# vovw/algonauts-2025

Hardware: AMD Instinct MI355X
Metric: TRs/sec trimodal encode to 1000 parcels (higher is better)
Workload: dtype bf16; 1 GPU; trimodal encode, precomputed bf16 feats, per GPU B=64 sequences (4 subjects x R=16) x T=1024, L*D=4096 per modality, hidden 3072, 8 layers, V=1000 parcels, n_output_timesteps=1024; forward only; global_batch=64, seq_len=1024, parallelism=dp1

## Files before the change

### algonauts-2025_amd/csrc/gemm.hip

```cpp
#include "gemm_common.h"

namespace {

constexpr int BK = 64;
typedef __attribute__((ext_vector_type(4))) short s16x4_tn;
constexpr int TRIBE_ROLE_EXT = 100;

namespace big {
constexpr int BM = 256, BN = 256;
constexpr int A_BYTES = BM * BK * 2;
constexpr int BUF_BYTES = 2 * A_BYTES;
constexpr int SMEM_BYTES = 2 * BUF_BYTES;
}

#define TRIBE_WAIT_VMCNT_(n) asm volatile("s_waitcnt vmcnt(" #n ")" ::: "memory")
#define TRIBE_WAIT_VMCNT(n) TRIBE_WAIT_VMCNT_(n)
#ifndef TRIBE_GEMM_VM_STEADY
#define TRIBE_GEMM_VM_STEADY 8
#endif

#ifdef TRIBE_GEMM_STAMPS
#define TRIBE_STAMP(var)                                                                  \
  do {                                                                                    \
    __builtin_amdgcn_sched_barrier(0);                                                    \
    asm volatile("s_memtime %0\n\ts_waitcnt lgkmcnt(0)" : "=s"(var)::"memory");           \
    __builtin_amdgcn_sched_barrier(0);                                                    \
  } while (0)
#define TRIBE_STAMP_ACC(slot, t_from, t_to) stamp_acc[slot] += (t_to) - (t_from)
#else
#define TRIBE_STAMP(var) do { } while (0)
#define TRIBE_STAMP_ACC(slot, t_from, t_to) do { } while (0)
#endif

template <int N> __device__ __forceinline__ void wait_vmcnt() { asm volatile("s_waitcnt vmcnt(%0)" ::"n"(N) : "memory"); }

struct SkSched {
  int tiles_dp;
  int rem_units;
  int q;
  int workers;
  float* ws;
  unsigned short second_worker[256];
};
constexpr int SK_SLOT_FLOATS = 256 * 256;

template <int OUT_BF16, int ROLE, int TN = 0, int NB = 4>
__global__ __launch_bounds__(512, 2) void gemm_nt_256x256x64(const tribe_gemm_desc g, int tiles_m, int tiles_n, const SkSched sk) {
  static_assert(NB >= 2 && NB <= 4 && (!TN || NB == 4), "tile columns: 128, 192 or 256; transposed operands: 256 only");
  constexpr int BM = big::BM, BN = 64 * NB, A_BYTES = big::A_BYTES, BUF_BYTES = A_BYTES + BN * BK * 2;
  constexpr int WN = 16 * NB;
  constexpr int VM_STEADY = NB == 4 ? TRIBE_GEMM_VM_STEADY : 4 + NB;
  extern __shared__ __attribute__((aligned(16))) char smem[];
#ifdef TRIBE_GEMM_STAMPS
  unsigned long long ts_entry = 0, ts_loop = 0, ts_end = 0;
  TRIBE_STAMP(ts_entry);
#endif
  const int tid = threadIdx.x;
  const int lane = tid & 63;
  const int wave = __builtin_amdgcn_readfirstlane(tid >> 6);
  const int wr = wave >> 2, wc = wave & 3;

  int tile_lin = (int)blockIdx.x, k_first = 0, nk = (int)(g.K / BK);
  bool partial = false;
  int sk_slot = 0;
  if constexpr (TN) {
    if ((int)blockIdx.x >= sk.tiles_dp) {
      const int sidx = (int)blockIdx.x - sk.tiles_dp;
      const bool second = sidx >= sk.workers;
      const int w = second ? (int)sk.second_worker[sidx - sk.workers] : sidx;
      const int u0 = w * sk.q;
      if (u0 >= sk.rem_units) return;
      const int run = min(sk.q, sk.rem_units - u0);
      const int t_loc = u0 / nk, x = u0 - t_loc * nk, first_len = min(run, nk - x);
      if (second && first_len >= run) return;
      tile_lin = sk.tiles_dp + t_loc + (second ? 1 : 0);
      k_first = second ? 0 : x;
      const int len = second ? run - first_len : first_len;
      partial = len != nk;
      nk = len;
      sk_slot = 2 * w + (second ? 1 : 0);
    }
  }
  int tm, tn;
  tile_coords(tile_lin, tiles_m, tiles_n, tm, tn);
  const int64_t m0 = (int64_t)tm * BM, n0 = (int64_t)tn * BN;

  const int64_t z = blockIdx.y;
  const int64_t b1 = z / g.batch0, b0 = z - b1 * g.batch0;
  const int64_t b1g = g.gather1 ? g.gather1[b1] : b1;
  const unsigned short* A = (const unsigned short*)g.A + (g.gather_a ? b1g : b1) * g.sA1 + b0 * g.sA0;
  const unsigned short* B = (const unsigned short*)g.B + (g.gather_b ? b1g : b1) * g.sB1 + b0 * g.sB0;

  const int srow = lane >> 3;
  const int schunk = (lane & 7) ^ srow;
#ifdef TRIBE_ABL_SAME_TILE
#define m0 ((int64_t)0)
#define n0 ((int64_t)0)
#endif
  const unsigned short* a_src[2][2];
  const unsigned short* b_src[NB];
  int a_lds[2][2], b_lds[NB];
#pragma unroll
  for (int h = 0; h < 2; ++h)
#pragma unroll
    for (int j = 0; j < 2; ++j) {
      if (TN) {
        const int piece = 8 * j + wave, krow = 4 * piece + (lane >> 4);
        const int lc = (lane & 15) ^ ((krow & 7) << 1);
        int64_t gm = m0 + (lc >> 3) * 128 + h * 64 + (lc & 7) * 8; gm = gm + 8 <= g.M ? gm : g.M - 8;
        int64_t gn = n0 + (lc >> 2) * 64 + h * 32 + (lc & 3) * 8; gn = gn + 8 <= g.N ? gn : g.N - 8;
        a_src[h][j] = A + (int64_t)krow * g.lda + gm;
        b_src[(2 * h + j) % NB] = B + (int64_t)krow * g.ldb + gn;
        a_lds[h][j] = h * 16384 + piece * 1024;
        b_lds[(2 * h + j) % NB] = A_BYTES + h * 16384 + piece * 1024;
      } else {
        const int ra = j * 128 + h * 64 + wave * 8;
        int64_t gr = m0 + ra + srow; gr = gr < g.M ? gr : g.M - 1;
        a_src[h][j] = A + gr * g.lda + schunk * 8;
        a_lds[h][j] = ra * 128;
      }
    }
  if (!TN) {
#pragma unroll
    for (int q = 0; q < NB; ++q) {
      const int rb = q * 64 + wave * 8;
      int64_t gc = n0 + rb + srow; gc = gc < g.N ? gc : g.N - 1;
      b_src[q] = B + gc * g.ldb + schunk * 8;
      b_lds[q] = A_BYTES + rb * 128;
    }
  }

#ifdef TRIBE_ABL_SAME_TILE
#undef m0
#undef n0
#endif
  auto stage = [&](int which, int buf, int kt) {
#ifdef TRIBE_ABL_NO_STAGE
    return;
#endif
    char* base = smem + buf * BUF_BYTES;
    const int64_t koff_a = TN ? (int64_t)kt * BK * g.lda : (int64_t)kt * BK;
    const int64_t koff_b = TN ? (int64_t)kt * BK * g.ldb : (int64_t)kt * BK;
    if (which == 0 || which == 3) {
      const int h = which == 3;
      __builtin_amdgcn_global_load_lds((gptr_t)(a_src[h][0] + koff_a), (lptr_t)(base + a_lds[h][0]), 16, 0, 0);
      __builtin_amdgcn_global_load_lds((gptr_t)(a_src[h][1] + koff_a), (lptr_t)(base + a_lds[h][1]), 16, 0, 0);
    } else {
#pragma unroll
      for (int q = 0; q < NB; ++q)
        __builtin_amdgcn_global_load_lds((gptr_t)(b_src[q] + koff_b), (lptr_t)(base + b_lds[q]), 16, 0, 0);
    }
  };

  f32x4_t acc[8][NB];
#pragma unroll
  for (int i = 0; i < 8; ++i)
#pragma unroll
    for (int j = 0; j < NB; ++j) acc[i][j] = f32x4_t{0.f, 0.f, 0.f, 0.f};

  const int frow = lane & 15, fq = lane >> 4;
  const int coff0 = ((fq ^ (frow & 7)) << 4), coff1 = (((4 + fq) ^ (frow & 7)) << 4);
  const int a_rd = (wr * 128 + frow) * 128;
#ifdef TRIBE_GEMM_NO_TACC
  constexpr int TACC = 0;
#else
  constexpr int TACC = TN ? 0 : 1;
#endif
  const int prow = TACC ? ((frow & 3) | ((frow & 4) << 1) | ((frow & 8) >> 1)) : frow;
  const int bcoff0 = ((fq ^ (prow & 7)) << 4), bcoff1 = (((4 + fq) ^ (prow & 7)) << 4);
  const int b_rd = A_BYTES + (wc * WN + prow) * 128;

  bf16x8_t fa[4][2], fb[NB][2];
#ifdef TRIBE_ABL_NO_LDSREAD
#pragma unroll
  for (int i = 0; i < 4; ++i)
#pragma unroll
    for (int k = 0; k < 2; ++k) {
      fa[i][k] = bf16x8_t{(short)(0x3c00 + lane), (short)0x3f80, (short)(0xbf00 + i), (short)0x3e00, (short)0xbe80, (short)0x3f00, (short)(0x3d00 + k), (short)0xbd00};
      if (i < NB) fb[i][k] = fa[i][k];
    }
#endif

  const int tq = frow >> 2, tp = frow & 3;
  const int t_row = 4 * fq + tq, t_sw = (t_row & 7) << 1;
  int ta_off[4], tb_off[2];
#pragma unroll
  for (int i = 0; i < 4; ++i) ta_off[i] = t_row * 256 + (((wr * 8 + 2 * i + (tp >> 1)) ^ t_sw) << 4) + (tp & 1) * 8;
#pragma unroll
  for (int j = 0; j < 2; ++j) tb_off[j] = A_BYTES + t_row * 256 + (((wc * 4 + 2 * j + (tp >> 1)) ^ t_sw) << 4) + (tp & 1) * 8;
  auto tr_frag = [&](const char* p) -> bf16x8_t {
    const s16x4_tn lo = __builtin_amdgcn_ds_read_tr16_b64_v4i16((__attribute__((address_space(3))) s16x4_tn*)(p));
    const s16x4_tn hi = __builtin_amdgcn_ds_read_tr16_b64_v4i16((__attribute__((address_space(3))) s16x4_tn*)(p + 16 * 256));
    bf16x8_t f;
#pragma unroll
    for (int e = 0; e < 4; ++e) { f[e] = lo[e]; f[4 + e] = hi[e]; }
    return f;
  };

#ifdef TRIBE_ABL_NO_LDSREAD
#define TRIBE_LDS_A(base, MH) _Pragma("unroll") for (int i = 0; i < 4; ++i) { asm volatile("" : "+v"(fa[i][0]), "+v"(fa[i][1])); }
#define TRIBE_LDS_B(base) _Pragma("unroll") for (int j = 0; j < NB; ++j) { asm volatile("" : "+v"(fb[j][0]), "+v"(fb[j][1])); }
#else
#define TRIBE_LDS_A(base, MH)                                                                  \
  _Pragma("unroll") for (int i = 0; i < 4; ++i) {                                              \
    if (TN) {                                                                                  \
      fa[i][0] = tr_frag((base) + (MH) * 16384 + ta_off[i]);                                   \
      fa[i][1] = tr_frag((base) + (MH) * 16384 + ta_off[i] + 32 * 256);                        \
    } else {                                                                                   \
      fa[i][0] = *(const bf16x8_t*)((base) + a_rd + (MH) * 8192 + i * 2048 + coff0);           \
      fa[i][1] = *(const bf16x8_t*)((base) + a_rd + (MH) * 8192 + i * 2048 + coff1);           \
    }                                                                                          \
  }
// ... 23 lines not shown
  }
#endif
#ifdef TRIBE_GEMM_PRIO_FLIPS
#define TRIBE_PRIO_UP() __builtin_amdgcn_s_setprio(1)
#define TRIBE_PRIO_DOWN() __builtin_amdgcn_s_setprio(0)
#else
#define TRIBE_PRIO_UP() __builtin_amdgcn_sched_barrier(0)
#define TRIBE_PRIO_DOWN() __builtin_amdgcn_sched_barrier(0)
#endif
#define TRIBE_PHASE_SYNC_MMA(MH)                           \
  asm volatile("s_waitcnt lgkmcnt(0)" ::: "memory");       \
  __builtin_amdgcn_sched_barrier(0);                       \
  TRIBE_STAMP(ts2);                                        \
  __builtin_amdgcn_s_barrier();                            \
  TRIBE_STAMP(ts3);                                        \
  TRIBE_PRIO_UP();                                         \
  TRIBE_MMA(MH)                                            \
  TRIBE_PRIO_DOWN();                                       \
  TRIBE_STAMP(ts4);                                        \
  __builtin_amdgcn_s_barrier();                            \
  TRIBE_STAMP(ts5);                                        \
  TRIBE_STAMP_ACC(1, ts1, ts2); TRIBE_STAMP_ACC(2, ts2, ts3); TRIBE_STAMP_ACC(3, ts3, ts4); TRIBE_STAMP_ACC(4, ts4, ts5);

#ifdef TRIBE_GEMM_NO_KROT
  const int krot = 0;
#else
  const int krot = ((tn & 7) + (tm & 3)) % nk;
#endif
  auto ktile = [&](int t) { const int k = t + krot; return k_first + (k >= nk ? k - nk : k); };
#ifdef TRIBE_GEMM_STAMPS
  unsigned long long ts0 = 0, ts1 = 0, ts2 = 0, ts3 = 0, ts4 = 0, ts5 = 0;
  unsigned long long stamp_acc[5] = {0, 0, 0, 0, 0};
#endif

  stage(0, 0, ktile(0)); stage(1, 0, ktile(0)); stage(3, 0, ktile(0));
  if (nk > 1) {
    stage(0, 1, ktile(1)); stage(1, 1, ktile(1));
    wait_vmcnt<2 + NB>();
  } else {
    wait_vmcnt<0>();
  }
  __builtin_amdgcn_s_barrier();
  if (wr == 1) __builtin_amdgcn_s_barrier();
#if !defined(TRIBE_GEMM_PRIO_FLIPS) && !defined(TRIBE_ABL_NO_PRIO)
  if (wr == 1) __builtin_amdgcn_s_setprio(1);
#endif

  TRIBE_STAMP(ts_loop);
  for (int t = 0; t < nk; ++t) {
    const int cur = t & 1;
    const char* base = smem + cur * BUF_BYTES;
    TRIBE_STAMP(ts0);
    TRIBE_LDS_B(base)
    TRIBE_LDS_A(base, 0)
    TRIBE_STAMP(ts1);
    TRIBE_STAMP_ACC(0, ts0, ts1);
    if (t + 1 < nk) { stage(3, cur ^ 1, ktile(t + 1)); wait_vmcnt<VM_STEADY>(); } else { wait_vmcnt<0>(); }
    TRIBE_PHASE_SYNC_MMA(0)
    TRIBE_STAMP(ts0);
    TRIBE_LDS_A(base, 1)
    TRIBE_STAMP(ts1);
    TRIBE_STAMP_ACC(0, ts0, ts1);
    if (t + 2 < nk) {
      const int k2 = ktile(t + 2);
// ... 9 lines not shown
  TRIBE_STAMP(ts_end);
#ifdef TRIBE_GEMM_STAMPS
  if (g.gadd == nullptr && g.gadd_index != nullptr && lane == 0 && blockIdx.y == 0) {
    unsigned long long* dbg = (unsigned long long*)g.gadd_index + ((size_t)blockIdx.x * 8 + wave) * 8;
    for (int i = 0; i < 5; ++i) dbg[i] = stamp_acc[i];
  }
#endif
#undef TRIBE_LDS_A
#undef TRIBE_LDS_B
#undef TRIBE_MMA
#undef TRIBE_PHASE_SYNC_MMA

  const EpiCtx ctx = make_epi_ctx(g, b1, b0, b1g);
  if constexpr (TN && !OUT_BF16) {
    if (partial) {
      float* slot = sk.ws + (int64_t)sk_slot * SK_SLOT_FLOATS + tid * 4;
      static_for<8 * NB>([&](auto t) {
        constexpr int i = decltype(t)::value / NB, j = decltype(t)::value % NB;
        *(f32x4_t*)(slot + (i * NB + j) * 2048) = acc[i][j];
      });
      return;
    }
  }
  constexpr bool ROLE_EPI = TACC && (ROLE == TRIBE_ROLE_QKV || ROLE == TRIBE_ROLE_FF1 || ROLE == TRIBE_ROLE_OUT_PROJ || ROLE == TRIBE_ROLE_FF2);
  if constexpr (ROLE_EPI) {
    epilogue_role<OUT_BF16, ROLE, 8, NB, TACC>(g, acc, m0 + wr * 128, n0 + wc * WN, lane, smem + wave * (4 * NB * 1024));
  } else if (epilogue_fast_ok<(ROLE == TRIBE_ROLE_EXT)>(g, ctx) && n0 + BN <= g.N) {
    epilogue_fast<OUT_BF16, 8, NB, (ROLE == TRIBE_ROLE_EXT), TACC>(g, ctx, acc, m0 + wr * 128, n0 + wc * WN, lane, smem + wave * (4 * NB * 1024));
  } else {
    static_for<8 * NB>([&](auto t) {
      constexpr int i = decltype(t)::value / NB, j = decltype(t)::value % NB;
      epilogue_tile16<OUT_BF16, (ROLE == TRIBE_ROLE_EXT), TACC>(g, ctx, acc[i][j], m0 + wr * 128 + i * 16, n0 + wc * WN + j * 16, lane);
    });
  }
#ifdef TRIBE_GEMM_STAMPS
  TRIBE_STAMP(ts1);
  asm volatile("s_waitcnt vmcnt(0)" ::: "memory");
  TRIBE_STAMP(ts2);
  if (g.gadd == nullptr && g.gadd_index != nullptr && lane == 0 && blockIdx.y == 0) {
    unsigned long long* dbg = (unsigned long long*)g.gadd_index + ((size_t)blockIdx.x * 8 + wave) * 8;
    dbg[5] = ts_loop - ts_entry; dbg[6] = ts1 - ts_end; dbg[7] = ts2 - ts_end;
  }
#endif
}

__global__ __launch_bounds__(512) void streamk_reduce_kernel(const tribe_gemm_desc g, int tiles_m, int tiles_n, const SkSched sk) {
  const int tid = threadIdx.x, lane = tid & 63, wave = tid >> 6, wr = wave >> 2, wc = wave & 3;
// ... 614 lines not shown




#ifndef TRIBE_GEMM_PART
#define TRIBE_GEMM_PART -1
#endif
#define TRIBE_GEMM_HAS_PART(p) (TRIBE_GEMM_PART < 0 || TRIBE_GEMM_PART == (p))

namespace tribe_gemm_detail {
enum { KIND_SMALL = 0, KIND_BIG = 1, KIND_RING = 2, KIND_BIG4W = 3 };
#define TRIBE_GEMM_PAIRS(X)                                                                                            \
  X(0, 1, TRIBE_ROLE_GENERIC) X(1, 0, TRIBE_ROLE_GENERIC) X(2, 1, TRIBE_ROLE_EXT) X(3, 0, TRIBE_ROLE_EXT)              \
  X(4, 0, TRIBE_ROLE_PROJECTOR) X(5, 1, TRIBE_ROLE_QKV) X(6, 0, TRIBE_ROLE_ATTN_SCORES) X(7, 1, TRIBE_ROLE_ATTN_PV)    \
  X(8, 0, TRIBE_ROLE_OUT_PROJ) X(9, 1, TRIBE_ROLE_FF1) X(10, 0, TRIBE_ROLE_FF2) X(11, 0, TRIBE_ROLE_VOXEL_HEAD)
void launch_big4(int pair, dim3 grid, hipStream_t s, const tribe_gemm_desc* d, int tiles_m, int tiles_n);
void launch_big4_tn(int bf, dim3 grid, hipStream_t s, const tribe_gemm_desc* d, int tiles_m, int tiles_n, const SkSched& sk);
void launch_big3(int pair, dim3 grid, hipStream_t s, const tribe_gemm_desc* d, int tiles_m, int tiles_n);
void launch_ring(int pair, dim3 grid, hipStream_t s, const tribe_gemm_desc* d, int tiles_m, int tiles_n, int splits, float* ws);
void launch_splitk_epilogue(int bf, hipStream_t s, const tribe_gemm_desc* d, int splits, const float* ws);
void launch_4w(int pair, dim3 grid, hipStream_t s, const tribe_gemm_desc* d, int tiles_m, int tiles_n);
void launch_small(int pair, dim3 grid, hipStream_t s, const tribe_gemm_desc* d, int tiles_m, int tiles_n);

template <auto KERNEL, int THREADS, int SMEM, class... Extra>
static void launch_k(dim3 grid, hipStream_t s, const tribe_gemm_desc* d, int tiles_m, int tiles_n, const Extra&... extra) {
  static bool attr_done[64] = {};
  int dev = 0;
  (void)hipGetDevice(&dev);
  if (dev < 0 || dev >= 64 || !attr_done[dev]) {
    (void)hipFuncSetAttribute((const void*)KERNEL, hipFuncAttributeMaxDynamicSharedMemorySize, SMEM);
    if (dev >= 0 && dev < 64) attr_done[dev] = true;
  }
  hipLaunchKernelGGL(KERNEL, grid, dim3(THREADS, 1, 1), SMEM, s, *d, tiles_m, tiles_n, extra...);
}
inline const SkSched& no_stream_k() {
  static const SkSched none = [] { SkSched k{}; k.tiles_dp = 0x7fffffff; return k; }();
  return none;
}
#define TRIBE_GEMM_TABLE(NAME)                                                                                         \
  void NAME(int pair, dim3 grid, hipStream_t s, const tribe_gemm_desc* d, int tiles_m, int tiles_n) {                  \
    switch (pair) {                                                                                                    \
      TRIBE_GEMM_PAIRS(TRIBE_GEMM_CASE_##NAME)                                                                         \
      default: break;                                                                                                  \
    }                                                                                                                  \
  }
#if TRIBE_GEMM_HAS_PART(0)
#define TRIBE_GEMM_CASE_launch_big4(idx, bf, role) \
  case idx: launch_k<gemm_nt_256x256x64<bf, role, 0, 4>, 512, big::SMEM_BYTES>(grid, s, d, tiles_m, tiles_n, no_stream_k()); break;
TRIBE_GEMM_TABLE(launch_big4)
void launch_big4_tn(int bf, dim3 grid, hipStream_t s, const tribe_gemm_desc* d, int tiles_m, int tiles_n, const SkSched& sk) {
  if (bf) launch_k<gemm_nt_256x256x64<1, TRIBE_ROLE_GENERIC, 1, 4>, 512, big::SMEM_BYTES>(grid, s, d, tiles_m, tiles_n, sk);
  else launch_k<gemm_nt_256x256x64<0, TRIBE_ROLE_GENERIC, 1, 4>, 512, big::SMEM_BYTES>(grid, s, d, tiles_m, tiles_n, sk);
}
#endif
#if TRIBE_GEMM_HAS_PART(1)
#define TRIBE_GEMM_CASE_launch_big3(idx, bf, role) \
  case idx: launch_k<gemm_nt_256x256x64<bf, role, 0, 3>, 512, 2 * (big::A_BYTES + 192 * BK * 2)>(grid, s, d, tiles_m, tiles_n, no_stream_k()); break;
TRIBE_GEMM_TABLE(launch_big3)
#endif
#if TRIBE_GEMM_HAS_PART(2)
#define TRIBE_GEMM_CASE_launch_ring(idx, bf, role) \
  case idx: launch_k<gemm_nt_ring128<bf, role>, 512, ring::SMEM_BYTES>(grid, s, d, tiles_m, tiles_n, splits, ws); break;
void launch_ring(int pair, dim3 grid, hipStream_t s, const tribe_gemm_desc* d, int tiles_m, int tiles_n, int splits, float* ws) {
  switch (pair) {
    TRIBE_GEMM_PAIRS(TRIBE_GEMM_CASE_launch_ring)
    default: break;
  }
}
void launch_splitk_epilogue(int bf, hipStream_t s, const tribe_gemm_desc* d, int splits, const float* ws) {
  const int64_t threads = d->M * (d->N / 4);
  const dim3 grid((unsigned)((threads + 255) / 256));
  if (bf) hipLaunchKernelGGL(splitk_epilogue_kernel<1>, grid, dim3(256), 0, s, *d, splits, ws);
  else hipLaunchKernelGGL(splitk_epilogue_kernel<0>, grid, dim3(256), 0, s, *d, splits, ws);
}
#define TRIBE_GEMM_CASE_launch_small(idx, bf, role) \
  case idx: launch_k<gemm_nt_128x128x64<bf, role>, 256, small::SMEM_BYTES>(grid, s, d, tiles_m, tiles_n); break;
TRIBE_GEMM_TABLE(launch_small)
#endif
#if TRIBE_GEMM_HAS_PART(3)
#ifdef TRIBE_GEMM_STAMPS4W
// ... 268 lines not shown
    TRIBE_REQUIRE(nz == 1 && !d->rowadd && !d->gadd && !d->aux && (d->act == TRIBE_ACT_NONE || d->act == TRIBE_ACT_GELU),
                  "tribe_gemm_bf16: c_bf16 / row_sumsq / row_scale need an un-batched launch with plain operators");
    TRIBE_REQUIRE(d->ldc % 4 == 0 && ((uintptr_t)d->C % 16) == 0 && (!d->bias || ((uintptr_t)d->bias % 16) == 0) &&
                      (!d->res || (d->ldres % 4 == 0 && ((uintptr_t)d->res % 16) == 0)) && (!d->res_scale || ((uintptr_t)d->res_scale % 16) == 0),
                  "tribe_gemm_bf16: c_bf16 / row_sumsq / row_scale need 16-byte aligned operands");
    TRIBE_REQUIRE((!d->c_bf16 && !d->row_sumsq) || d->c_dtype == TRIBE_F32, "tribe_gemm_bf16: c_bf16 / row_sumsq accompany an f32 C");
    TRIBE_REQUIRE(!d->c_bf16 || (d->ld_c_bf16 >= d->N && d->ld_c_bf16 % 4 == 0 && ((uintptr_t)d->c_bf16 % 8) == 0), "tribe_gemm_bf16: bad c_bf16");
  }
  const tribe_gemm_detail::GemmPlan plan = tribe_gemm_detail::gemm_plan(d);
  if (d->c_bf16 || d->row_sumsq || d->row_scale) {
    TRIBE_REQUIRE(d->N % plan.bn == 0, "tribe_gemm_bf16: c_bf16 / row_sumsq / row_scale need N (%lld) to be a multiple of the tile width %d",
                  (long long)d->N, plan.bn);
    TRIBE_REQUIRE(!d->row_sumsq || d->ld_row_sumsq >= d->N / plan.sumsq_cols, "tribe_gemm_bf16: ld_row_sumsq must cover N / %d slots (tribe_gemm_sumsq_slots)",
                  plan.sumsq_cols);
  }
  if (d->trans_ab) {
    TRIBE_REQUIRE(d->M >= 8 && d->N >= 8 && d->M % 8 == 0 && d->N % 8 == 0 && d->lda >= d->M && d->ldb >= d->N,
                  "tribe_gemm_bf16: trans_ab takes At [K, M] and Bt [K, N] with M and N multiples of 8 and lda >= M, ldb >= N");
    TRIBE_REQUIRE(!d->aux && d->act != TRIBE_ACT_SWIGLU && d->act != TRIBE_ACT_GLU && d->act != TRIBE_ACT_SILU && d->act != TRIBE_ACT_GELU_BWD &&
                      d->act != TRIBE_ACT_EXP2 && d->act != TRIBE_ACT_MUL_AUX && !d->gather_a && !d->gather_b,
                  "tribe_gemm_bf16: trans_ab supports the plain epilogue operators and no operand gather");
  }
  const int64_t tiles_m = (d->M + plan.bm - 1) / plan.bm, tiles_n = (d->N + plan.bn - 1) / plan.bn;
  TRIBE_REQUIRE(tiles_m * tiles_n < (1ll << 31) && nz < 65536, "tribe_gemm_bf16: grid too large");

  dim3 grid((unsigned)(tiles_m * tiles_n), (unsigned)nz, 1);
  hipStream_t s = (hipStream_t)stream;
  const int role = (d->role >= 0 && d->role < TRIBE_ROLE_COUNT) ? d->role : TRIBE_ROLE_GENERIC;
  const double flops = 2.0 * (double)d->M * (double)d->N * (double)d->K * (double)nz;
  const int slot = prof_before(role, flops, s);
  const bool bf = d->c_dtype == TRIBE_BF16;
  if (d->trans_ab) {
    SkSched sk = tribe_gemm_detail::no_stream_k();
    if (d->stream_k) {
      TRIBE_REQUIRE(!bf && nz == 1 && d->bias_mode == TRIBE_BIAS_NONE && d->act == TRIBE_ACT_NONE && !d->res && !d->rowadd && !d->gadd,
                    "tribe_gemm_bf16: stream_k takes a plain un-batched f32 product");
      grid.x = tribe_gemm_detail::plan_stream_k((int)(tiles_m * tiles_n), (int)(d->K / BK), &sk);
      if (sk.tiles_dp < tiles_m * tiles_n) {
        const int64_t need = (int64_t)2 * sk.workers * SK_SLOT_FLOATS * 4;
        TRIBE_REQUIRE(d->stream_k_ws && d->stream_k_ws_bytes >= need && ((uintptr_t)d->stream_k_ws % 16) == 0,
                      "tribe_gemm_bf16: stream_k needs a 16-byte aligned workspace of %lld bytes (tribe_gemm_stream_k_workspace_bytes)", (long long)need);
        sk.ws = (float*)d->stream_k_ws;
      }
    }
    tribe_gemm_detail::launch_big4_tn(bf ? 1 : 0, grid, s, d, (int)tiles_m, (int)tiles_n, sk);
    if (sk.tiles_dp < tiles_m * tiles_n)
      hipLaunchKernelGGL(streamk_reduce_kernel, dim3((unsigned)(tiles_m * tiles_n - sk.tiles_dp)), dim3(512), 0, s, *d, (int)tiles_m, (int)tiles_n, sk);
// ... 19 lines not shown
    default: break;
    }
  }
  using namespace tribe_gemm_detail;
  if (plan.kind == KIND_BIG && (pair == 5 || pair == 8 || pair == 9 || pair == 10) && !takes_role_epilogue(d, plan)) pair = bf ? 0 : 1;
  if (plan.kind == KIND_BIG4W) launch_4w(pair, grid, s, d, (int)tiles_m, (int)tiles_n);
  else if (plan.kind == KIND_BIG && plan.bn == 192) launch_big3(pair, grid, s, d, (int)tiles_m, (int)tiles_n);
  else if (plan.kind == KIND_BIG) launch_big4(pair, grid, s, d, (int)tiles_m, (int)tiles_n);
  else if (plan.kind == KIND_RING && plan.splits > 1) {
    const int64_t need = (int64_t)plan.splits * d->M * d->N * 4;
    TRIBE_REQUIRE(d->stream_k_ws && d->stream_k_ws_bytes >= need && ((uintptr_t)d->stream_k_ws % 16) == 0,
                  "tribe_gemm_bf16: this launch is split over K: stream_k_ws must hold %lld bytes (tribe_gemm_stream_k_workspace_bytes)", (long long)need);
    TRIBE_REQUIRE(tiles_m * tiles_n * plan.splits < (1ll << 31) && d->M * (d->N / 4) < (1ll << 39), "tribe_gemm_bf16: grid too large");
    grid.x = (unsigned)(tiles_m * tiles_n * plan.splits);
    launch_ring(pair, grid, s, d, (int)tiles_m, (int)tiles_n, plan.splits, (float*)d->stream_k_ws);
    launch_splitk_epilogue(bf ? 1 : 0, s, d, plan.splits, (const float*)d->stream_k_ws);
  } else if (plan.kind == KIND_RING) launch_ring(pair, grid, s, d, (int)tiles_m, (int)tiles_n, 1, nullptr);
  else launch_small(pair, grid, s, d, (int)tiles_m, (int)tiles_n);
  prof_after(slot, s);
  TRIBE_LAUNCH_CHECK();
  return 0;
}

extern "C" int tribe_gemm_stream_k_plan(int32_t tiles, int32_t nk, int32_t* out) {
  TRIBE_REQUIRE(tiles > 0 && nk > 0 && out != nullptr, "tribe_gemm_stream_k_plan: bad argument");
  SkSched sk;
  const unsigned grid = tribe_gemm_detail::plan_stream_k(tiles, nk, &sk);
  out[0] = sk.tiles_dp; out[1] = sk.rem_units; out[2] = sk.q; out[3] = sk.workers;
  for (int i = 0; i < 256; ++i) out[4 + i] = sk.second_worker[i];
  return (int)grid;
}

extern "C" int64_t tribe_gemm_stream_k_workspace_bytes(const tribe_gemm_desc* d) {
  TRIBE_REQUIRE(d != nullptr && d->M > 0 && d->N > 0 && d->K > 0 && d->K % BK == 0, "tribe_gemm_stream_k_workspace_bytes: bad descriptor");
  if (!d->stream_k || d->batch1 * d->batch0 != 1) return 0;
  if (!d->trans_ab) {
    const tribe_gemm_detail::GemmPlan plan = tribe_gemm_detail::gemm_plan(d);
    return plan.splits > 1 ? (int64_t)plan.splits * d->M * d->N * 4 : 0;
  }
  SkSched sk;
  const int tiles = (int)(((d->M + 255) / 256) * ((d->N + 255) / 256));
  if (tribe_gemm_detail::plan_stream_k(tiles, (int)(d->K / BK), &sk) == (unsigned)tiles) return 0;
  return (int64_t)2 * sk.workers * SK_SLOT_FLOATS * 4;
}

extern "C" int tribe_gemm_sumsq_slots(const tribe_gemm_desc* d) {
// ... 13 lines not shown
```

### algonauts-2025_amd/csrc/gemm_common.h

```cpp
#pragma once
#include "common.h"
#include <utility>

typedef const __attribute__((address_space(1))) void* gptr_t;
typedef __attribute__((address_space(3))) void* lptr_t;

__device__ __forceinline__ float gelu_erf(float x) {
  return 0.5f * x * (1.0f + erff(x * 0.70710678118654752440f));
}

__device__ __forceinline__ int xcd_remap(int bid, int nwg) {
  const int q = nwg >> 3, r = nwg & 7, xcd = bid & 7;
  const int base = (xcd < r) ? xcd * (q + 1) : r * (q + 1) + (xcd - r) * q;
  return base + (bid >> 3);
}

__device__ __forceinline__ void tile_coords(int bid, int tiles_m, int tiles_n, int& tm, int& tn) {
#ifndef TRIBE_GEMM_BAND_ROWS
#define TRIBE_GEMM_BAND_ROWS 4
#endif
  constexpr int GM = TRIBE_GEMM_BAND_ROWS;
  const int tile = xcd_remap(bid, tiles_m * tiles_n);
  const int band = tile / (GM * tiles_n);
  const int first_m = band * GM;
  const int gm = (tiles_m - first_m < GM) ? tiles_m - first_m : GM;
  const int r = tile - band * GM * tiles_n;
  tn = r / gm;
  tm = first_m + (r - tn * gm);
}

typedef __attribute__((ext_vector_type(2))) float f32x2_t;
__device__ __forceinline__ f32x2_t gelu_poly2(f32x2_t v) {
  f32x2_t c;
  c.x = __builtin_amdgcn_fmed3f(v.x, -4.4f, 4.4f);
  c.y = __builtin_amdgcn_fmed3f(v.y, -4.4f, 4.4f);
  const f32x2_t t = c * c;
  f32x2_t q = 4.4347532590638394e-11f;
  q = q * t + -4.493755145773548e-09f;
  q = q * t + 2.0033526482166053e-07f;
  q = q * t + -5.224721007834887e-06f;
  q = q * t + 8.98004655027762e-05f;
  q = q * t + -0.0010902436915785074f;
  q = q * t + 0.009767354466021061f;
  q = q * t + -0.06628739088773727f;
  q = q * t + 0.3988831341266632f;
  const f32x2_t phi = c * q + 0.5f;
  return v * phi;
}

__device__ __forceinline__ float gelu_grad(float v) {
  const float cdf = 0.5f * (1.0f + erff(v * 0.70710678118654752440f));
  const float pdf = 0.3989422804014327f * __expf(-0.5f * v * v);
// ... 513 lines not shown
```

### algonauts-2025_amd/tribe_hip/_lib.py

```python

from __future__ import annotations

import ctypes as C
import os
from pathlib import Path

import numpy as _np

_HERE = Path(__file__).resolve().parent
LIB_PATH = _HERE / "libtribe_hip.so"

F32, BF16, F64 = 0, 1, 2
ACT_NONE, ACT_GELU, ACT_SWIGLU, ACT_SILU, ACT_GLU, ACT_GELU_BWD, ACT_EXP2, ACT_MUL_AUX = 0, 1, 2, 3, 4, 5, 6, 7
BIAS_NONE, BIAS_COL, BIAS_ROW = 0, 1, 2
ROLES = ["generic", "projector", "qkv", "attn_scores", "attn_pv", "out_proj", "ff1", "ff2", "voxel_head", "attention"]
ROLE = {name: index for index, name in enumerate(ROLES)}

i64, i32, f32, vp, sz = C.c_int64, C.c_int32, C.c_float, C.c_void_p, C.c_size_t


ADAM_TENSOR_DTYPE = _np.dtype([("p", "<u8"), ("g", "<u8"), ("m", "<u8"), ("v", "<u8"), ("n", "<i8"), ("p_bf16", "<u8")], align=True)
FEATURE_PIECE_DTYPE = _np.dtype([("src", "<u8"), ("ld", "<i8"), ("src_first", "<i4"), ("src_count", "<i4"), ("dst_first", "<i4"),
                                 ("dst_count", "<i4")], align=True)

# ... 128 lines not shown
        ("final_norm_g", vp),
        ("cos_tab", vp), ("sin_tab", vp),
    ]


ABI_VERSION = 5
STRUCT_MIRRORS = [
    ("tribe_gemm_desc", GemmDesc), ("tribe_attention_desc", AttentionDesc), ("tribe_encoder_layer", EncoderLayer), ("tribe_encoder_desc", EncoderDesc),
    ("tribe_vit_layer", VitLayer), ("tribe_vit_fp8_layer", VitFp8Layer), ("tribe_vjepa2_desc", Vjepa2Desc), ("tribe_conformer_layer", ConformerLayer),
    ("tribe_conformer_fp8_layer", ConformerFp8Layer), ("tribe_w2vbert_desc", W2vBertDesc), ("tribe_llama_layer", LlamaLayer),
    ("tribe_llama_fp8_layer", LlamaFp8Layer), ("tribe_llama_desc", LlamaDesc), ("tribe_feature_piece", FEATURE_PIECE_DTYPE),
    ("tribe_adam_tensor", ADAM_TENSOR_DTYPE),
]

SIGNATURES = {
    "tribe_version": (C.c_int, []),
    "tribe_abi_struct_sizes": (C.c_int, [C.POINTER(i64), i32]),
    "tribe_last_error": (C.c_char_p, []),
    "tribe_gemm_bf16": (C.c_int, [C.POINTER(GemmDesc), vp]),
    "tribe_gemm_sumsq_slots": (C.c_int, [C.POINTER(GemmDesc)]),
    "tribe_gemm_epilogue_path": (C.c_int, [C.POINTER(GemmDesc)]),
    "tribe_gemm_stream_k_workspace_bytes": (i64, [C.POINTER(GemmDesc)]),
    "tribe_gemm_stream_k_plan": (C.c_int, [i32, i32, C.POINTER(i32)]),
    "tribe_prof_begin": (C.c_int, [i32]),
    "tribe_prof_end": (C.c_int, [i32, C.POINTER(C.c_double), C.POINTER(i64), C.POINTER(C.c_double)]),
    "tribe_pack_weight_bf16": (C.c_int, [vp, i64, i64, i64, vp, i64, i64, vp]),
    "tribe_pack_subject_weights": (C.c_int, [vp, i64, i64, i64, vp, i64, i64, vp]),
    "tribe_pack_features": (C.c_int, [vp, i32, i64, i64, i64, i64, i32, vp, i64, vp]),
    "tribe_projector_fwd": (C.c_int, [vp, i64, i64, i64, vp, vp, i64, vp, i64, i64, i32, vp, vp, vp, vp]),
    "tribe_projector_zero_fwd": (C.c_int, [i64, i64, i64, vp, i64, i64, vp, vp, vp, vp]),
    "tribe_scalenorm_fwd": (C.c_int, [vp, i64, i64, vp, f32, f32, vp, i32, vp]),
    "tribe_rotary_fwd": (C.c_int, [vp, i64, i64, i64, i32, i32, i32, vp, vp, i32, vp]),
    "tribe_attention_fwd_ex": (C.c_int, [C.POINTER(AttentionDesc), vp]),
    "tribe_embedding_fwd": (C.c_int, [vp, i32, vp, i64, i64, i64, vp, vp]),
    "tribe_rmsnorm_fwd": (C.c_int, [vp, i64, i64, vp, f32, vp, i32, vp]),
    "tribe_layernorm_fwd": (C.c_int, [vp, i64, i64, vp, vp, f32, vp, i32, vp]),
    "tribe_segment_mean_fwd": (C.c_int, [vp, i64, i64, i64, vp, vp, vp, i64, vp]),
    "tribe_window_mean_fwd": (C.c_int, [vp, i64, i64, i64, vp, vp, vp, i64, vp, i64, vp]),
    "tribe_im2col3d_fwd": (C.c_int, [vp, i64, i32, i32, i32, i32, i32, i32, vp, i64, vp]),
    "tribe_vjepa2_workspace_bytes": (sz, [C.POINTER(Vjepa2Desc)]),
    "tribe_vjepa2_fwd": (C.c_int, [C.POINTER(Vjepa2Desc), vp, vp, sz, vp]),
    "tribe_dwconv_ln_swish_fwd": (C.c_int, [vp, i64, i64, i32, i32, vp, vp, vp, f32, vp, vp]),
    "tribe_gather_rows_fwd": (C.c_int, [vp, i64, i64, i64, vp, i64, vp, vp]),
    "tribe_w2vbert_workspace_bytes": (sz, [C.POINTER(W2vBertDesc)]),
    "tribe_w2vbert_fwd": (C.c_int, [C.POINTER(W2vBertDesc), vp, vp, sz, vp]),
    "tribe_transpose_bf16": (C.c_int, [vp, i32, i64, i64, i64, i64, i64, vp, i64, i64, vp]),
# ... 109 lines not shown
```

### include/tribe_hip.h

```cpp
#ifndef TRIBE_HIP_H
#define TRIBE_HIP_H

#include <stddef.h>
#include <stdint.h>

#ifdef __cplusplus
extern "C" {
#endif

#define TRIBE_ABI_VERSION 5

enum tribe_dtype { TRIBE_F32 = 0, TRIBE_BF16 = 1, TRIBE_F64 = 2 };
enum tribe_act {
  TRIBE_ACT_NONE = 0,
  TRIBE_ACT_GELU = 1,
  TRIBE_ACT_SWIGLU = 2,
  TRIBE_ACT_SILU = 3,
  TRIBE_ACT_GLU = 4,
  TRIBE_ACT_GELU_BWD = 5,
  TRIBE_ACT_EXP2 = 6,
  TRIBE_ACT_MUL_AUX = 7
};
enum tribe_bias_mode { TRIBE_BIAS_NONE = 0, TRIBE_BIAS_COL = 1, TRIBE_BIAS_ROW = 2 };
enum tribe_gemm_role {
// ... 21 lines not shown
  int32_t act;
  const float* res; int64_t ldres, sRes1, sRes0;
  const float* res_scale;
  const float* rowadd; int64_t ld_rowadd, rowadd_period;
  const float* gadd; const int64_t* gadd_index; int64_t gadd_div, ld_gadd;
  void* aux; int64_t ld_aux;
  int32_t gather_b;
  int32_t role;
  int32_t tile_hint;
  int32_t trans_ab;
  uint16_t* c_bf16; int64_t ld_c_bf16;
  float* row_sumsq; int64_t ld_row_sumsq;
  const float* row_scale;
  int64_t sBias0;
  int32_t stream_k; int32_t reserved0;
  void* stream_k_ws; int64_t stream_k_ws_bytes;
} tribe_gemm_desc;

int tribe_gemm_bf16(const tribe_gemm_desc* desc, void* stream);
int tribe_gemm_sumsq_slots(const tribe_gemm_desc* desc);
int tribe_gemm_epilogue_path(const tribe_gemm_desc* desc);
int64_t tribe_gemm_stream_k_workspace_bytes(const tribe_gemm_desc* desc);
int tribe_gemm_stream_k_plan(int32_t tiles, int32_t nk, int32_t* out);
int tribe_rownorm_scale_fwd(const float* partial, int64_t rows, int64_t n_partial, const float* g, float gain_scale, float eps,
                            float* scale, void* stream);

int tribe_rowdot_heads_bf16(const uint16_t* a, int64_t ld_a, const uint16_t* b, int64_t ld_b, int64_t B, int64_t T, int32_t heads, int32_t dim_head,
                            float scale, float* out, void* stream);

int tribe_prof_begin(int32_t max_records);
int tribe_prof_end(int32_t n_roles, double* total_ms_host, int64_t* count_host, double* flops_host);

int tribe_pack_weight_bf16(const float* src, int64_t rows, int64_t cols, int64_t ld_src,
                           uint16_t* dst, int64_t rows_pad, int64_t cols_pad, void* stream);
int tribe_pack_subject_weights(const float* w, int64_t S, int64_t C, int64_t V,
                               uint16_t* dst, int64_t V_pad, int64_t C_pad, void* stream);

int tribe_pack_features(const void* feat, int32_t dtype, int64_t B, int64_t L, int64_t D, int64_t T,
                        int32_t layer_mean, uint16_t* dst, int64_t K_pad, void* stream);

int tribe_projector_fwd(const uint16_t* feat_packed, int64_t BT, int64_t T, int64_t K_pad,
                        const uint16_t* w_packed , const float* bias , int64_t N_out,
                        float* x, int64_t hidden, int64_t col0, int32_t accumulate,
                        const float* pos_embed ,
                        const float* subj_embed , const int64_t* subject_id ,
                        void* stream);
// ... 301 lines not shown
```

Measured before the change: 639,800 TRs/s.

## Precompute GEMM kernel prologue on host and issue first loads before accumulator setup

Adds a host-computed GemmHead kernel argument holding base pointers, strides, k-tile count, a reciprocal for the k-rotation modulo and a precomputed tile-walk structure, so the big GEMM kernel avoids integer divisions and descriptor decoding in its prologue. Batch offset math is skipped for unbatched and role-epilogue launches. The first global-to-LDS stage loads are now issued before the accumulator zeroing and fragment offset setup, with sched barriers and asm pins, to overlap prologue latency. It increases kernel argument size and adds code complexity, plus a host-side tile_walk helper for testing.

```diff
diff --git a/algonauts-2025_amd/csrc/gemm.hip b/algonauts-2025_amd/csrc/gemm.hip
--- a/algonauts-2025_amd/csrc/gemm.hip
+++ b/algonauts-2025_amd/csrc/gemm.hip
@@ -45,7 +45,7 @@
 constexpr int SK_SLOT_FLOATS = 256 * 256;
 
 template <int OUT_BF16, int ROLE, int TN = 0, int NB = 4>
-__global__ __launch_bounds__(512, 2) void gemm_nt_256x256x64(const tribe_gemm_desc g, int tiles_m, int tiles_n, const SkSched sk) {
+__global__ __launch_bounds__(512, 2) void gemm_nt_256x256x64(const GemmHead hd, const tribe_gemm_desc g, const SkSched sk) {
   static_assert(NB >= 2 && NB <= 4 && (!TN || NB == 4), "tile columns: 128, 192 or 256; transposed operands: 256 only");
   constexpr int BM = big::BM, BN = 64 * NB, A_BYTES = big::A_BYTES, BUF_BYTES = A_BYTES + BN * BK * 2;
   constexpr int WN = 16 * NB;
@@ -60,7 +60,7 @@
   const int wave = __builtin_amdgcn_readfirstlane(tid >> 6);
   const int wr = wave >> 2, wc = wave & 3;
 
-  int tile_lin = (int)blockIdx.x, k_first = 0, nk = (int)(g.K / BK);
+  int tile_lin = (int)blockIdx.x, k_first = 0, nk = hd.nk;
   bool partial = false;
   int sk_slot = 0;
   if constexpr (TN) {
@@ -82,14 +82,28 @@
     }
   }
   int tm, tn;
-  tile_coords(tile_lin, tiles_m, tiles_n, tm, tn);
+  if constexpr (TN) tile_coords(tile_lin, hd.walk.tiles_m, hd.walk.tiles_n, tm, tn);
+  else tile_walk_coords(hd.walk, tile_lin, tm, tn);
   const int64_t m0 = (int64_t)tm * BM, n0 = (int64_t)tn * BN;
 
-  const int64_t z = blockIdx.y;
-  const int64_t b1 = z / g.batch0, b0 = z - b1 * g.batch0;
-  const int64_t b1g = g.gather1 ? g.gather1[b1] : b1;
-  const unsigned short* A = (const unsigned short*)g.A + (g.gather_a ? b1g : b1) * g.sA1 + b0 * g.sA0;
-  const unsigned short* B = (const unsigned short*)g.B + (g.gather_b ? b1g : b1) * g.sB1 + b0 * g.sB0;
+#ifdef TRIBE_GEMM_NO_TACC
+  constexpr int TACC = 0;
+#else
+  constexpr int TACC = TN ? 0 : 1;
+#endif
+  constexpr bool ROLE_EPI = TACC && (ROLE == TRIBE_ROLE_QKV || ROLE == TRIBE_ROLE_FF1 || ROLE == TRIBE_ROLE_OUT_PROJ || ROLE == TRIBE_ROLE_FF2);
+  int64_t b1 = 0, b0 = 0, b1g = 0;
+  const unsigned short* A = hd.A;
+  const unsigned short* B = hd.B;
+  if constexpr (!ROLE_EPI) {
+    if (hd.batched) {
+      const int64_t z = blockIdx.y;
+      b1 = z / g.batch0; b0 = z - b1 * g.batch0;
+      b1g = g.gather1 ? g.gather1[b1] : b1;
+      A += (g.gather_a ? b1g : b1) * g.sA1 + b0 * g.sA0;
+      B += (g.gather_b ? b1g : b1) * g.sB1 + b0 * g.sB0;
+    }
+  }
 
   const int srow = lane >> 3;
   const int schunk = (lane & 7) ^ srow;
@@ -100,6 +114,9 @@
   const unsigned short* a_src[2][2];
   const unsigned short* b_src[NB];
   int a_lds[2][2], b_lds[NB];
+  const unsigned short* a_tile = A + m0 * hd.lda;
+  const unsigned short* b_tile = B + n0 * hd.ldb;
+  const int m_last = (int)(hd.M - 1 - m0 < BM - 1 ? hd.M - 1 - m0 : BM - 1), n_last = (int)(hd.N - 1 - n0 < BN - 1 ? hd.N - 1 - n0 : BN - 1);
 #pragma unroll
   for (int h = 0; h < 2; ++h)
 #pragma unroll
@@ -107,16 +124,16 @@
       if (TN) {
         const int piece = 8 * j + wave, krow = 4 * piece + (lane >> 4);
         const int lc = (lane & 15) ^ ((krow & 7) << 1);
-        int64_t gm = m0 + (lc >> 3) * 128 + h * 64 + (lc & 7) * 8; gm = gm + 8 <= g.M ? gm : g.M - 8;
-        int64_t gn = n0 + (lc >> 2) * 64 + h * 32 + (lc & 3) * 8; gn = gn + 8 <= g.N ? gn : g.N - 8;
-        a_src[h][j] = A + (int64_t)krow * g.lda + gm;
-        b_src[(2 * h + j) % NB] = B + (int64_t)krow * g.ldb + gn;
+        int64_t gm = m0 + (lc >> 3) * 128 + h * 64 + (lc & 7) * 8; gm = gm + 8 <= hd.M ? gm : hd.M - 8;
+        int64_t gn = n0 + (lc >> 2) * 64 + h * 32 + (lc & 3) * 8; gn = gn + 8 <= hd.N ? gn : hd.N - 8;
+        a_src[h][j] = A + (int64_t)krow * hd.lda + gm;
+        b_src[(2 * h + j) % NB] = B + (int64_t)krow * hd.ldb + gn;
         a_lds[h][j] = h * 16384 + piece * 1024;
         b_lds[(2 * h + j) % NB] = A_BYTES + h * 16384 + piece * 1024;
       } else {
         const int ra = j * 128 + h * 64 + wave * 8;
-        int64_t gr = m0 + ra + srow; gr = gr < g.M ? gr : g.M - 1;
-        a_src[h][j] = A + gr * g.lda + schunk * 8;
+        const int rel = min(ra + srow, m_last);
+        a_src[h][j] = a_tile + (int64_t)(uint64_t)(unsigned)rel * hd.lda + schunk * 8;
         a_lds[h][j] = ra * 128;
       }
     }
@@ -124,8 +141,8 @@
 #pragma unroll
     for (int q = 0; q < NB; ++q) {
       const int rb = q * 64 + wave * 8;
-      int64_t gc = n0 + rb + srow; gc = gc < g.N ? gc : g.N - 1;
-      b_src[q] = B + gc * g.ldb + schunk * 8;
+      const int rel = min(rb + srow, n_last);
+      b_src[q] = b_tile + (int64_t)(uint64_t)(unsigned)rel * hd.ldb + schunk * 8;
       b_lds[q] = A_BYTES + rb * 128;
     }
   }
@@ -139,8 +156,8 @@
     return;
 #endif
     char* base = smem + buf * BUF_BYTES;
-    const int64_t koff_a = TN ? (int64_t)kt * BK * g.lda : (int64_t)kt * BK;
-    const int64_t koff_b = TN ? (int64_t)kt * BK * g.ldb : (int64_t)kt * BK;
+    const int64_t koff_a = TN ? (int64_t)kt * BK * hd.lda : (int64_t)kt * BK;
+    const int64_t koff_b = TN ? (int64_t)kt * BK * hd.ldb : (int64_t)kt * BK;
     if (which == 0 || which == 3) {
       const int h = which == 3;
       __builtin_amdgcn_global_load_lds((gptr_t)(a_src[h][0] + koff_a), (lptr_t)(base + a_lds[h][0]), 16, 0, 0);
@@ -152,23 +169,33 @@
     }
   };
 
+#ifdef TRIBE_GEMM_NO_KROT
+  const int krot = 0;
+#else
+  const int krot_x = (tn & 7) + (tm & 3);
+  const int krot = TN ? krot_x % nk : krot_x - nk * (int)(((unsigned)krot_x * hd.krot_rcp) >> 16);
+#endif
+  auto ktile = [&](int t) { const int k = t + krot; return k_first + (k >= nk ? k - nk : k); };
+
+  stage(0, 0, ktile(0)); stage(1, 0, ktile(0)); stage(3, 0, ktile(0));
+  if (nk > 1) { stage(0, 1, ktile(1)); stage(1, 1, ktile(1)); }
+  __builtin_amdgcn_sched_barrier(0);
+
   f32x4_t acc[8][NB];
 #pragma unroll
   for (int i = 0; i < 8; ++i)
 #pragma unroll
-    for (int j = 0; j < NB; ++j) acc[i][j] = f32x4_t{0.f, 0.f, 0.f, 0.f};
+    for (int j = 0; j < NB; ++j) {
+      acc[i][j] = f32x4_t{0.f, 0.f, 0.f, 0.f};
+      asm volatile("" : "+v"(acc[i][j]));
+    }
 
   const int frow = lane & 15, fq = lane >> 4;
-  const int coff0 = ((fq ^ (frow & 7)) << 4), coff1 = (((4 + fq) ^ (frow & 7)) << 4);
-  const int a_rd = (wr * 128 + frow) * 128;
-#ifdef TRIBE_GEMM_NO_TACC
-  constexpr int TACC = 0;
-#else
-  constexpr int TACC = TN ? 0 : 1;
-#endif
+  int coff0_ = ((fq ^ (frow & 7)) << 4), coff1_ = (((4 + fq) ^ (frow & 7)) << 4);
+  int a_rd_ = (wr * 128 + frow) * 128;
   const int prow = TACC ? ((frow & 3) | ((frow & 4) << 1) | ((frow & 8) >> 1)) : frow;
-  const int bcoff0 = ((fq ^ (prow & 7)) << 4), bcoff1 = (((4 + fq) ^ (prow & 7)) << 4);
-  const int b_rd = A_BYTES + (wc * WN + prow) * 128;
+  int bcoff0_ = ((fq ^ (prow & 7)) << 4), bcoff1_ = (((4 + fq) ^ (prow & 7)) << 4);
+  int b_rd_ = A_BYTES + (wc * WN + prow) * 128;
 
   bf16x8_t fa[4][2], fb[NB][2];
 #ifdef TRIBE_ABL_NO_LDSREAD
@@ -188,6 +215,12 @@
   for (int i = 0; i < 4; ++i) ta_off[i] = t_row * 256 + (((wr * 8 + 2 * i + (tp >> 1)) ^ t_sw) << 4) + (tp & 1) * 8;
 #pragma unroll
   for (int j = 0; j < 2; ++j) tb_off[j] = A_BYTES + t_row * 256 + (((wc * 4 + 2 * j + (tp >> 1)) ^ t_sw) << 4) + (tp & 1) * 8;
+  if constexpr (TN) {
+    asm volatile("" : "+v"(ta_off[0]), "+v"(ta_off[1]), "+v"(ta_off[2]), "+v"(ta_off[3]), "+v"(tb_off[0]), "+v"(tb_off[1]));
+  } else {
+    asm volatile("" : "+v"(a_rd_), "+v"(coff0_), "+v"(coff1_), "+v"(b_rd_), "+v"(bcoff0_), "+v"(bcoff1_));
+  }
+  const int a_rd = a_rd_, coff0 = coff0_, coff1 = coff1_, b_rd = b_rd_, bcoff0 = bcoff0_, bcoff1 = bcoff1_;
   auto tr_frag = [&](const char* p) -> bf16x8_t {
     const s16x4_tn lo = __builtin_amdgcn_ds_read_tr16_b64_v4i16((__attribute__((address_space(3))) s16x4_tn*)(p));
     const s16x4_tn hi = __builtin_amdgcn_ds_read_tr16_b64_v4i16((__attribute__((address_space(3))) s16x4_tn*)(p + 16 * 256));
@@ -257,24 +290,13 @@
   TRIBE_STAMP(ts5);                                        \
   TRIBE_STAMP_ACC(1, ts1, ts2); TRIBE_STAMP_ACC(2, ts2, ts3); TRIBE_STAMP_ACC(3, ts3, ts4); TRIBE_STAMP_ACC(4, ts4, ts5);
 
-#ifdef TRIBE_GEMM_NO_KROT
-  const int krot = 0;
-#else
-  const int krot = ((tn & 7) + (tm & 3)) % nk;
-#endif
-  auto ktile = [&](int t) { const int k = t + krot; return k_first + (k >= nk ? k - nk : k); };
 #ifdef TRIBE_GEMM_STAMPS
   unsigned long long ts0 = 0, ts1 = 0, ts2 = 0, ts3 = 0, ts4 = 0, ts5 = 0;
   unsigned long long stamp_acc[5] = {0, 0, 0, 0, 0};
 #endif
 
-  stage(0, 0, ktile(0)); stage(1, 0, ktile(0)); stage(3, 0, ktile(0));
-  if (nk > 1) {
-    stage(0, 1, ktile(1)); stage(1, 1, ktile(1));
-    wait_vmcnt<2 + NB>();
-  } else {
-    wait_vmcnt<0>();
-  }
+  __builtin_amdgcn_sched_barrier(0);
+  if (nk > 1) wait_vmcnt<2 + NB>(); else wait_vmcnt<0>();
   __builtin_amdgcn_s_barrier();
   if (wr == 1) __builtin_amdgcn_s_barrier();
 #if !defined(TRIBE_GEMM_PRIO_FLIPS) && !defined(TRIBE_ABL_NO_PRIO)
@@ -330,7 +352,6 @@
       return;
     }
   }
-  constexpr bool ROLE_EPI = TACC && (ROLE == TRIBE_ROLE_QKV || ROLE == TRIBE_ROLE_FF1 || ROLE == TRIBE_ROLE_OUT_PROJ || ROLE == TRIBE_ROLE_FF2);
   if constexpr (ROLE_EPI) {
     epilogue_role<OUT_BF16, ROLE, 8, NB, TACC>(g, acc, m0 + wr * 128, n0 + wc * WN, lane, smem + wave * (4 * NB * 1024));
   } else if (epilogue_fast_ok<(ROLE == TRIBE_ROLE_EXT)>(g, ctx) && n0 + BN <= g.N) {
@@ -991,8 +1012,8 @@
 void launch_4w(int pair, dim3 grid, hipStream_t s, const tribe_gemm_desc* d, int tiles_m, int tiles_n);
 void launch_small(int pair, dim3 grid, hipStream_t s, const tribe_gemm_desc* d, int tiles_m, int tiles_n);
 
-template <auto KERNEL, int THREADS, int SMEM, class... Extra>
-static void launch_k(dim3 grid, hipStream_t s, const tribe_gemm_desc* d, int tiles_m, int tiles_n, const Extra&... extra) {
+template <auto KERNEL, int SMEM>
+static void allow_dynamic_lds() {
   static bool attr_done[64] = {};
   int dev = 0;
   (void)hipGetDevice(&dev);
@@ -1000,11 +1021,30 @@
     (void)hipFuncSetAttribute((const void*)KERNEL, hipFuncAttributeMaxDynamicSharedMemorySize, SMEM);
     if (dev >= 0 && dev < 64) attr_done[dev] = true;
   }
+}
+template <auto KERNEL, int THREADS, int SMEM, class... Extra>
+static void launch_k(dim3 grid, hipStream_t s, const tribe_gemm_desc* d, int tiles_m, int tiles_n, const Extra&... extra) {
+  allow_dynamic_lds<KERNEL, SMEM>();
   hipLaunchKernelGGL(KERNEL, grid, dim3(THREADS, 1, 1), SMEM, s, *d, tiles_m, tiles_n, extra...);
 }
 inline const SkSched& no_stream_k() {
   static const SkSched none = [] { SkSched k{}; k.tiles_dp = 0x7fffffff; return k; }();
   return none;
+}
+inline GemmHead gemm_head(const tribe_gemm_desc* d, int tiles_m, int tiles_n) {
+  GemmHead h;
+  h.A = (const unsigned short*)d->A; h.B = (const unsigned short*)d->B;
+  h.lda = d->lda; h.ldb = d->ldb; h.M = d->M; h.N = d->N;
+  h.nk = (int)(d->K / BK);
+  h.krot_rcp = (unsigned)(65536 / h.nk + 1);
+  h.batched = (d->batch1 * d->batch0 != 1 || d->gather1) ? 1 : 0;
+  h.walk = make_tile_walk(tiles_m, tiles_n);
+  return h;
+}
+template <auto KERNEL, int SMEM>
+static void launch_big(dim3 grid, hipStream_t s, const tribe_gemm_desc* d, int tiles_m, int tiles_n, const SkSched& sk) {
+  allow_dynamic_lds<KERNEL, SMEM>();
+  hipLaunchKernelGGL(KERNEL, grid, dim3(512, 1, 1), SMEM, s, gemm_head(d, tiles_m, tiles_n), *d, sk);
 }
 #define TRIBE_GEMM_TABLE(NAME)                                                                                         \
   void NAME(int pair, dim3 grid, hipStream_t s, const tribe_gemm_desc* d, int tiles_m, int tiles_n) {                  \
@@ -1015,16 +1055,16 @@
   }
 #if TRIBE_GEMM_HAS_PART(0)
 #define TRIBE_GEMM_CASE_launch_big4(idx, bf, role) \
-  case idx: launch_k<gemm_nt_256x256x64<bf, role, 0, 4>, 512, big::SMEM_BYTES>(grid, s, d, tiles_m, tiles_n, no_stream_k()); break;
+  case idx: launch_big<gemm_nt_256x256x64<bf, role, 0, 4>, big::SMEM_BYTES>(grid, s, d, tiles_m, tiles_n, no_stream_k()); break;
 TRIBE_GEMM_TABLE(launch_big4)
 void launch_big4_tn(int bf, dim3 grid, hipStream_t s, const tribe_gemm_desc* d, int tiles_m, int tiles_n, const SkSched& sk) {
-  if (bf) launch_k<gemm_nt_256x256x64<1, TRIBE_ROLE_GENERIC, 1, 4>, 512, big::SMEM_BYTES>(grid, s, d, tiles_m, tiles_n, sk);
-  else launch_k<gemm_nt_256x256x64<0, TRIBE_ROLE_GENERIC, 1, 4>, 512, big::SMEM_BYTES>(grid, s, d, tiles_m, tiles_n, sk);
+  if (bf) launch_big<gemm_nt_256x256x64<1, TRIBE_ROLE_GENERIC, 1, 4>, big::SMEM_BYTES>(grid, s, d, tiles_m, tiles_n, sk);
+  else launch_big<gemm_nt_256x256x64<0, TRIBE_ROLE_GENERIC, 1, 4>, big::SMEM_BYTES>(grid, s, d, tiles_m, tiles_n, sk);
 }
 #endif
 #if TRIBE_GEMM_HAS_PART(1)
 #define TRIBE_GEMM_CASE_launch_big3(idx, bf, role) \
-  case idx: launch_k<gemm_nt_256x256x64<bf, role, 0, 3>, 512, 2 * (big::A_BYTES + 192 * BK * 2)>(grid, s, d, tiles_m, tiles_n, no_stream_k()); break;
+  case idx: launch_big<gemm_nt_256x256x64<bf, role, 0, 3>, 2 * (big::A_BYTES + 192 * BK * 2)>(grid, s, d, tiles_m, tiles_n, no_stream_k()); break;
 TRIBE_GEMM_TABLE(launch_big3)
 #endif
 #if TRIBE_GEMM_HAS_PART(2)
@@ -1339,7 +1379,7 @@
                   "tribe_gemm_bf16: trans_ab supports the plain epilogue operators and no operand gather");
   }
   const int64_t tiles_m = (d->M + plan.bm - 1) / plan.bm, tiles_n = (d->N + plan.bn - 1) / plan.bn;
-  TRIBE_REQUIRE(tiles_m * tiles_n < (1ll << 31) && nz < 65536, "tribe_gemm_bf16: grid too large");
+  TRIBE_REQUIRE(tiles_m * tiles_n < (1ll << 31) && tiles_n < (1ll << 28) && nz < 65536, "tribe_gemm_bf16: grid too large");
 
   dim3 grid((unsigned)(tiles_m * tiles_n), (unsigned)nz, 1);
   hipStream_t s = (hipStream_t)stream;
@@ -1405,6 +1445,17 @@
   return 0;
 }
 
+extern "C" int tribe_gemm_tile_walk(int32_t tiles_m, int32_t tiles_n, int32_t bid, int32_t* tm, int32_t* tn) {
+  TRIBE_REQUIRE(tiles_m > 0 && tiles_n > 0 && (int64_t)tiles_m * tiles_n < (1ll << 31) && tiles_n < (1 << 28) && bid >= 0 &&
+                    bid < tiles_m * tiles_n && tm != nullptr && tn != nullptr,
+                "tribe_gemm_tile_walk: bad argument");
+  const TileWalk w = make_tile_walk(tiles_m, tiles_n);
+  int m = 0, n = 0;
+  tile_walk_coords(w, bid, m, n);
+  *tm = m; *tn = n;
+  return 0;
+}
+
 extern "C" int tribe_gemm_stream_k_plan(int32_t tiles, int32_t nk, int32_t* out) {
   TRIBE_REQUIRE(tiles > 0 && nk > 0 && out != nullptr, "tribe_gemm_stream_k_plan: bad argument");
   SkSched sk;
diff --git a/algonauts-2025_amd/csrc/gemm_common.h b/algonauts-2025_amd/csrc/gemm_common.h
--- a/algonauts-2025_amd/csrc/gemm_common.h
+++ b/algonauts-2025_amd/csrc/gemm_common.h
@@ -15,10 +15,10 @@
   return base + (bid >> 3);
 }
 
-__device__ __forceinline__ void tile_coords(int bid, int tiles_m, int tiles_n, int& tm, int& tn) {
 #ifndef TRIBE_GEMM_BAND_ROWS
 #define TRIBE_GEMM_BAND_ROWS 4
 #endif
+__device__ __forceinline__ void tile_coords(int bid, int tiles_m, int tiles_n, int& tm, int& tn) {
   constexpr int GM = TRIBE_GEMM_BAND_ROWS;
   const int tile = xcd_remap(bid, tiles_m * tiles_n);
   const int band = tile / (GM * tiles_n);
@@ -28,6 +28,67 @@
   tn = r / gm;
   tm = first_m + (r - tn * gm);
 }
+
+struct TileWalk {
+  int q, r;
+  int band;
+  unsigned band_rcp;
+  int band_shift;
+  int full_bands;
+  int last_gm;
+  int tiles_m, tiles_n;
+};
+
+__host__ __device__ inline TileWalk make_tile_walk(int tiles_m, int tiles_n) {
+  constexpr int GM = TRIBE_GEMM_BAND_ROWS;
+  TileWalk w;
+  const long long nwg = (long long)tiles_m * tiles_n;
+  w.tiles_m = tiles_m; w.tiles_n = tiles_n;
+  w.q = (int)(nwg >> 3); w.r = (int)(nwg & 7);
+  w.band = GM * tiles_n;
+  int s = 1;
+  while ((1ll << s) < (long long)w.band) ++s;
+  w.band_rcp = (unsigned)((1ull << (31 + s)) / (unsigned long long)w.band + 1ull);
+  w.band_shift = s - 1;
+  w.full_bands = tiles_m / GM;
+  w.last_gm = tiles_m % GM;
+  return w;
+}
+
+__host__ __device__ __forceinline__ void tile_walk_coords(const TileWalk& w, int bid, int& tm, int& tn) {
+  constexpr int GM = TRIBE_GEMM_BAND_ROWS;
+  static_assert((GM & (GM - 1)) == 0, "band height: a power of two");
+  const int xcd = bid & 7;
+  const unsigned tile = (unsigned)(xcd * w.q + (xcd < w.r ? xcd : w.r) + (bid >> 3));
+  const unsigned band = (unsigned)(((unsigned long long)tile * w.band_rcp) >> 32) >> w.band_shift;
+  const unsigned r = tile - band * (unsigned)w.band;
+  if ((int)band < w.full_bands) {
+    tn = (int)(r / (unsigned)GM);
+    tm = (int)(band * GM + (r & (unsigned)(GM - 1)));
+  } else {
+    unsigned c;
+    if constexpr (GM == 4) {
+      const unsigned third = (unsigned)(((unsigned long long)r * 0xAAAAAAABull) >> 32) >> 1;
+      c = w.last_gm == 1 ? r : (w.last_gm == 2 ? r >> 1 : third);
+    } else {
+      c = r / (unsigned)w.last_gm;
+    }
+    tn = (int)c;
+    tm = (int)(band * GM + (r - c * (unsigned)w.last_gm));
+  }
+}
+
+struct GemmHead {
+  const unsigned short* A;
+  const unsigned short* B;
+  int64_t lda, ldb;
+  int64_t M, N;
+  TileWalk walk;
+  int nk;
+  unsigned krot_rcp;
+  int batched;
+};
+static_assert(sizeof(GemmHead) % 8 == 0, "the descriptor follows the head in the kernel-argument segment without padding");
 
 typedef __attribute__((ext_vector_type(2))) float f32x2_t;
 __device__ __forceinline__ f32x2_t gelu_poly2(f32x2_t v) {
diff --git a/algonauts-2025_amd/tribe_hip/_lib.py b/algonauts-2025_amd/tribe_hip/_lib.py
--- a/algonauts-2025_amd/tribe_hip/_lib.py
+++ b/algonauts-2025_amd/tribe_hip/_lib.py
@@ -174,6 +174,7 @@
     "tribe_gemm_epilogue_path": (C.c_int, [C.POINTER(GemmDesc)]),
     "tribe_gemm_stream_k_workspace_bytes": (i64, [C.POINTER(GemmDesc)]),
     "tribe_gemm_stream_k_plan": (C.c_int, [i32, i32, C.POINTER(i32)]),
+    "tribe_gemm_tile_walk": (C.c_int, [i32, i32, i32, C.POINTER(i32), C.POINTER(i32)]),
     "tribe_prof_begin": (C.c_int, [i32]),
     "tribe_prof_end": (C.c_int, [i32, C.POINTER(C.c_double), C.POINTER(i64), C.POINTER(C.c_double)]),
     "tribe_pack_weight_bf16": (C.c_int, [vp, i64, i64, i64, vp, i64, i64, vp]),
diff --git a/include/tribe_hip.h b/include/tribe_hip.h
--- a/include/tribe_hip.h
+++ b/include/tribe_hip.h
@@ -67,6 +67,7 @@
 int tribe_gemm_epilogue_path(const tribe_gemm_desc* desc);
 int64_t tribe_gemm_stream_k_workspace_bytes(const tribe_gemm_desc* desc);
 int tribe_gemm_stream_k_plan(int32_t tiles, int32_t nk, int32_t* out);
+int tribe_gemm_tile_walk(int32_t tiles_m, int32_t tiles_n, int32_t bid, int32_t* tm, int32_t* tn);
 int tribe_rownorm_scale_fwd(const float* partial, int64_t rows, int64_t n_partial, const float* g, float gain_scale, float eps,
                             float* scale, void* stream);
 
```

Measured after the change: 642,000 TRs/s, median of 6. No clear change (+0.3%).
